# cvg/glue-factory

Measured on AMD Instinct MI355X. Metric: image-pairs/sec (train step) SP+LightGlue N=2048 d=256 L=9, higher is better.
Workload: dtype bf16; 1 GPU; configs[1]: SuperPoint + LightGlue train step -- frozen SuperPoint-open forward on 2x32 synthetic 1024x1024 images resident in HBM (view1 = view0 warped by a sampled homography, SURVEY 8(d)(P); first block and the 64-channel 3x3 blocks as fused HIP kernels, library convolutions + fused HIP tails for the 128/256-channel blocks), homography ground truth (gf_gt_nn), LightGlue fwd + loss + bwd + fused; pairs_per_gpu=32, global_batch=32, keypoints=2048, descriptor_dim=256, layers=9, parallelism=dp1

## Files before the change

### glue-factory_amd/csrc/elementwise.hip

```cpp
#include "gf_common.h"
#include "gf_amd.h"

namespace {

typedef unsigned int u32x4_ __attribute__((ext_vector_type(4)));
__device__ __forceinline__ void load8(float (&x)[8], const bf16_t* p) {
    union { u32x4_ u; bf16_t e[8]; } v;
    v.u = *reinterpret_cast<const u32x4_*>(p);
#pragma unroll
    for (int e = 0; e < 8; ++e) x[e] = (float)v.e[e];
}
__device__ __forceinline__ void load8(float (&x)[8], const float* p) {
    const f32x4 a = *reinterpret_cast<const f32x4*>(p), b = *reinterpret_cast<const f32x4*>(p + 4);
#pragma unroll
    for (int e = 0; e < 4; ++e) { x[e] = a[e]; x[4 + e] = b[e]; }
}
__device__ __forceinline__ void store8(bf16_t* p, const float (&x)[8]) {
    union { u32x4_ u; bf16_t e[8]; } v;
#pragma unroll
    for (int e = 0; e < 8; ++e) v.e[e] = (bf16_t)x[e];
    *reinterpret_cast<u32x4_*>(p) = v.u;
}
__device__ __forceinline__ void store8(float* p, const float (&x)[8]) {
    f32x4 a = {x[0], x[1], x[2], x[3]}, b = {x[4], x[5], x[6], x[7]};
// ... 61 lines not shown
        }
        float acc[4], o[8];
#pragma unroll
        for (int i = 0; i < 4; ++i) {
            const float co = c[2 * i], si = INVERSE ? -c[2 * i + 1] : c[2 * i + 1];
            if (WITH_DTHETA) acc[i] = x[2 * i + 1] * y[2 * i] - x[2 * i] * y[2 * i + 1];
            o[2 * i] = x[2 * i] * co - x[2 * i + 1] * si;
            o[2 * i + 1] = x[2 * i + 1] * co + x[2 * i] * si;
        }
        if (active) store8(base, o);
        if (WITH_DTHETA) {
#pragma unroll
            for (int i = 0; i < 4; ++i)
                for (int off = cpd; off < 64; off <<= 1) acc[i] += __shfl_xor(acc[i], off);
            if (lane < cpd) {
                f32x4 v = {acc[0], acc[1], acc[2], acc[3]};
                if (dtheta_base) v += *reinterpret_cast<const f32x4*>(dtheta_base + tok * (D / 2) + lane * 4);
                *reinterpret_cast<f32x4*>(dtheta + tok * (D / 2) + lane * 4) = v;
            }
        }
    }
}

__device__ __forceinline__ void gelu_parts(float z, float& cdf, float& pdf) {
    const float x = fabsf(z) * 0.70710678118654752f;
    const float t = __builtin_amdgcn_rcpf(1.f + 0.3275911f * x);
    const float e = __expf(-x * x);
    const float poly = t * (0.254829592f + t * (-0.284496736f + t * (1.421413741f + t * (-1.453152027f + t * 1.061405429f))));
    const float erf_abs = 1.f - poly * e;
    cdf = 0.5f * (1.f + copysignf(erf_abs, z));
    pdf = 0.3989422804014327f * e;
}
__device__ __forceinline__ float gelu_f(float z) {
    float cdf, pdf;
    gelu_parts(z, cdf, pdf);
    return z * cdf;
}
__device__ __forceinline__ float gelu_grad(float z) {
    float cdf, pdf;
    gelu_parts(z, cdf, pdf);
    return cdf + z * pdf;
}

template <typename T> struct Chunk { static constexpr int VEC = 16 / sizeof(T); };
typedef unsigned int u32x4 __attribute__((ext_vector_type(4)));

template <typename T, int NCH, bool FULL = false>
__device__ __forceinline__ void load_row(float (&x)[NCH][16 / sizeof(T)], const T* row, int C, int lane) {
    constexpr int VEC = 16 / sizeof(T);
#pragma unroll
    for (int ch = 0; ch < NCH; ++ch) {
        int col = (ch * 64 + lane) * VEC;
        if (FULL || col < C) {
            union { u32x4 u; T e[VEC]; } v;
            v.u = *reinterpret_cast<const u32x4*>(row + col);
#pragma unroll
            for (int e = 0; e < VEC; ++e) x[ch][e] = to_f32(v.e[e]);
        } else {
#pragma unroll
            for (int e = 0; e < VEC; ++e) x[ch][e] = 0.f;
        }
    }
}
template <typename T, int NCH, bool FULL = false>
__device__ __forceinline__ void store_row(T* row, const float (&y)[NCH][16 / sizeof(T)], int C, int lane) {
    constexpr int VEC = 16 / sizeof(T);
// ... 22 lines not shown
            int col = (ch * 64 + lane) * VEC + e;
            g[ch][e] = (FULL || col < C) ? gamma[col] : 0.f;
            bt[ch][e] = (FULL || col < C) ? beta[col] : 0.f;
        }
    constexpr int RPI = 1;
    const int stride = gridDim.x * 4 * RPI;
    const float inv_c = 1.f / C;
    int row = (blockIdx.x * 4 + wave) * RPI;
    float nxt[RPI][NCH][VEC];
#pragma unroll
    for (int r = 0; r < RPI; ++r)
        if (row + r < R) load_row<T, NCH, FULL>(nxt[r], x + (int64_t)(row + r) * C, C, lane);
    for (; row < R; row += stride) {
        float v[RPI][NCH][VEC];
#pragma unroll
        for (int r = 0; r < RPI; ++r)
#pragma unroll
            for (int ch = 0; ch < NCH; ++ch)
#pragma unroll
                for (int e = 0; e < VEC; ++e) v[r][ch][e] = nxt[r][ch][e];
#pragma unroll
        for (int r = 0; r < RPI; ++r)
            if (row + stride + r < R) load_row<T, NCH, FULL>(nxt[r], x + (int64_t)(row + stride + r) * C, C, lane);
        float x0[RPI], s[RPI], q[RPI];
#pragma unroll
        for (int r = 0; r < RPI; ++r) {
            x0[r] = __builtin_bit_cast(float, __builtin_amdgcn_readlane(__builtin_bit_cast(int, v[r][0][0]), 0));
            s[r] = 0.f;
            q[r] = 0.f;
#pragma unroll
            for (int ch = 0; ch < NCH; ++ch)
#pragma unroll
                for (int e = 0; e < VEC; ++e) {
                    int col = (ch * 64 + lane) * VEC + e;
                    float d = (FULL || col < C) ? v[r][ch][e] - x0[r] : 0.f;
                    s[r] += d;
                    q[r] += d * d;
                }
        }
#pragma unroll
        for (int r = 0; r < RPI; ++r) {
            s[r] = wave_allsum(s[r]);
            q[r] = wave_allsum(q[r]);
        }
#pragma unroll
        for (int r = 0; r < RPI; ++r) {
            if (row + r >= R) break;
            const float md = s[r] * inv_c;
            const float mu = x0[r] + md;
            float var = fmaxf(q[r] * inv_c - md * md, 0.f);
            if (md * md > 63.f * var) {
                float q2 = 0.f;
#pragma unroll
                for (int ch = 0; ch < NCH; ++ch)
#pragma unroll
                    for (int e = 0; e < VEC; ++e) {
                        int col = (ch * 64 + lane) * VEC + e;
                        float dc = (FULL || col < C) ? (v[r][ch][e] - x0[r]) - md : 0.f;
                        q2 += dc * dc;
                    }
                var = wave_allsum(q2) * inv_c;
            }
            const float rs = rsqrtf(var + eps);
#pragma unroll
            for (int ch = 0; ch < NCH; ++ch)
#pragma unroll
                for (int e = 0; e < VEC; ++e)
                    v[r][ch][e] = gelu_f((v[r][ch][e] - mu) * rs * g[ch][e] + bt[ch][e]);
            store_row<T, NCH, FULL>(y + (int64_t)(row + r) * C, v[r], C, lane);
            if (lane == 0) { mean[row + r] = mu; rstd[row + r] = rs; }
        }
    }
}

template <typename T, int NCH, bool FULL>
__global__ __launch_bounds__(256) void ln_gelu_bwd_kernel(const T* x, const float* gamma, const float* beta,
                                                          const float* mean, const float* rstd, const T* dy, T* dx,
                                                          float* dgamma_part, float* dbeta_part, int R, int C) {
    constexpr int VEC = 16 / sizeof(T);
    extern __shared__ __attribute__((aligned(16))) char smem[];
    float* red = reinterpret_cast<float*>(smem);
    const int lane = threadIdx.x & 63, wave = threadIdx.x >> 6;
    float g[NCH][VEC], bt[NCH][VEC], dg[NCH][VEC], db[NCH][VEC];
#pragma unroll
    for (int ch = 0; ch < NCH; ++ch)
#pragma unroll
        for (int e = 0; e < VEC; ++e) {
            int col = (ch * 64 + lane) * VEC + e;
            g[ch][e] = (FULL || col < C) ? gamma[col] : 0.f;
            bt[ch][e] = (FULL || col < C) ? beta[col] : 0.f;
            dg[ch][e] = 0.f;
// ... 185 lines not shown
```

### glue-factory_amd/csrc/gemm_st.hip

```cpp
#include <type_traits>
#include "gf_common.h"
#include "gf_amd.h"

namespace {

typedef unsigned int u32x4 __attribute__((ext_vector_type(4)));
typedef unsigned int u32x2 __attribute__((ext_vector_type(2)));
typedef __attribute__((address_space(3))) void gs_lds_void;
typedef const __attribute__((address_space(1))) void gs_glb_void;

constexpr int GS_TILE = 32768;
#ifndef GS_NSTAGE_
#define GS_NSTAGE_ 3
#endif
#ifndef GS_WGS
#define GS_WGS 256
#endif
constexpr int GS_NSTAGE = GS_NSTAGE_, GS_PD = GS_NSTAGE - 1;

struct GsParams {
    const bf16_t* x0; const bf16_t* x1; const bf16_t* w; const float* bias; const bf16_t* res; const bf16_t* res2; bf16_t* y;
    const float* cs;
    int M, N;
    int64_t ld0, ld1, ldw, ldr, ldr2, ldy;
};

template <int OFF> __device__ __forceinline__ u32x4 gs_rd128(unsigned a) {
    u32x4 v;
    asm volatile("ds_read_b128 %0, %1 offset:%2" : "=v"(v) : "v"(a), "n"(OFF) : "memory");
    return v;
}
template <int N> __device__ __forceinline__ void gs_wait_lgkm() { asm volatile("s_waitcnt lgkmcnt(%0)" ::"n"(N) : "memory"); }
template <int N> __device__ __forceinline__ void gs_wait_vm() { asm volatile("s_waitcnt vmcnt(%0)" ::"n"(N) : "memory"); }
template <typename V> __device__ __forceinline__ void gs_tie(V& v) { asm volatile("" : "+v"(v)); }
__device__ __forceinline__ u32x4 gs_ld128(const void* p) {
    u32x4 v;
    asm volatile("global_load_dwordx4 %0, %1, off" : "=v"(v) : "v"(p) : "memory");
    return v;
}
__device__ __forceinline__ void gs_st128(void* p, u32x4 v) {
    asm volatile("global_store_dwordx4 %0, %1, off\n\ts_nop 2" ::"v"(p), "v"(v) : "memory");
}
__device__ __forceinline__ void gs_swap(unsigned& a, unsigned& b) {
    const auto r = __builtin_amdgcn_permlane32_swap(a, b, false, false);
    a = r[0]; b = r[1];
}

template <int KF, bool TWO, int RES, bool ROT>
__global__ __launch_bounds__(512, 2) void gemm_st_kernel(GsParams p) {
    extern __shared__ __attribute__((aligned(1024))) char smem[];
    constexpr int K = 16 * KF, ROWB = 2 * K, CPR = ROWB / 16;
    constexpr int TR = GS_TILE / ROWB, NRB = TR / 32;
    constexpr int NR = RES * 2 * NRB + (ROT ? 4 * NRB : 0), NS = 2 * NRB;
    const unsigned lds0 = (unsigned)(size_t)smem;
    const int lane = threadIdx.x & 63, wave = __builtin_amdgcn_readfirstlane(threadIdx.x >> 6);
    const int l31 = lane & 31, hi = lane >> 5;
    const int ch0 = blockIdx.y * 256 + wave * 32;
    const int ntile = p.M / TR;
    const int T = (ntile - (int)blockIdx.x + (int)gridDim.x - 1) / (int)gridDim.x;
    if (T <= 0) return;

    bf16x8 wf[KF];
#pragma unroll
    for (int s = 0; s < KF; ++s) wf[s] = *reinterpret_cast<const bf16x8*>(p.w + (int64_t)(ch0 + l31) * p.ldw + 16 * s + 8 * hi);
    float bias16[16];
#pragma unroll
    for (int r = 0; r < 16; ++r) bias16[r] = p.bias ? p.bias[ch0 + crow(r, hi)] : 0.f;
    gs_wait_vm<0>();

// ... 180 lines not shown
```

### glue-factory_amd/lib.py

```python
import ctypes
import os
import subprocess

_HERE = os.path.dirname(os.path.abspath(__file__))
LIB_PATH = os.path.join(_HERE, "libgf_amd.so")
CSRC = os.path.join(_HERE, "csrc")
ABI_VERSION = 20

_c = ctypes
_P, _I, _F, _L, _D = _c.c_void_p, _c.c_int, _c.c_float, _c.c_int64, _c.c_double
_S = _c.POINTER(_c.c_int64)

SIGNATURES = {
    "gf_abi_version": [],
    "gf_attn_fwd": [_P, _P, _P, _P, _P, _I, _I, _I, _I, _I, _S, _S, _S, _S, _F, _I, _P],
    "gf_attn_fwd_ex": [_P, _P, _P, _P, _P, _I, _I, _I, _I, _I, _S, _S, _S, _S, _F, _I, _I, _P, _P],
    "gf_attn_cross_bwd": [_P, _P, _P, _P, _P, _P, _P, _P, _I, _I, _I, _I, _I, _S, _S, _S, _S, _S, _S, _F, _I, _P],
    "gf_attn_bwd": [_P, _P, _P, _P, _P, _P, _P, _P, _P, _P, _I, _I, _I, _I, _I,
                    _S, _S, _S, _S, _S, _S, _S, _S, _F, _I, _P],
    "gf_attn_bwd_acc": [_P, _P, _P, _P, _P, _P, _P, _P, _P, _P, _I, _I, _I, _I, _I,
                        _S, _S, _S, _S, _S, _S, _S, _S, _F, _I, _I, _P],
    "gf_rows_lse": [_P, _P, _P, _P, _I, _I, _I, _I, _I, _P],
    "gf_rows_argmax": [_P, _P, _P, _F, _P, _P, _I, _I, _I, _I, _I, _P],
    "gf_assign_write": [_P, _P, _P, _P, _P, _P, _F, _F, _P, _P, _I, _I, _I, _I, _I, _P],
# ... 13 lines not shown
    "gf_line_segsum": [_P, _L, _P, _L, _P, _P, _P, _P, _I, _I, _I, _I, _I, _I, _P],
    "gf_line_expand": [_P, _P, _P, _P, _I, _I, _I, _I, _I, _I, _P],
    "gf_rows_gather": [_P, _P, _P, _I, _I, _I, _I, _I, _P],
    "gf_line_pair_scores": [_P, _P, _P, _I, _I, _I, _I, _P],
    "gf_dense_rowcol": [_P, _L, _L, _P, _P, _I, _I, _I, _I, _P],
    "gf_dense_assign": [_P, _P, _P, _P, _P, _F, _P, _I, _I, _I, _P],
    "gf_dense_assign_bwd": [_P, _P, _P, _P, _P, _P, _P, _I, _I, _I, _P],
    "gf_bgemm": [_P, _P, _P, _I, _I, _I, _I, _S, _S, _S, _F, _I, _P],
    "gf_multi_cast_transpose": [_P, _I, _I, _I, _P],
    "gf_cast_entry_bytes": [],
    "gf_fold_entry_bytes": [],
    "gf_fold_linear_fwd": [_P, _I, _I, _P],
    "gf_fold_linear_bwd": [_P, _P, _P, _P, _P, _P, _P, _P, _P, _I, _I, _I, _I, _I, _P],
    "gf_adam_entry_bytes": [],
    "gf_multi_adam": [_P, _I, _P, _P, _P, _P, _D, _D, _F, _F, _P],
    "gf_weight_grad_map": [_P, _P, _P, _P, _P, _F, _I, _I, _P],
    "gf_colsum_f32": [_P, _P, _P, _I, _I, _I, _P],
    "gf_colsum_ws_floats": [_I, _I],
    "gf_small_dw": [_P, _P, _P, _P, _I, _I, _I, _P],
    "gf_small_dw_ws_floats": [_I, _I],
    "gf_small_fwd": [_P, _P, _P, _I, _I, _I, _P],
    "gf_gemm": [_P, _P, _P, _P, _P, _P, _P, _I, _I, _I, _I, _I, _L, _L, _L, _L, _L, _I, _P],
    "gf_gemm_res2": [_P, _P, _P, _P, _P, _P, _P, _I, _I, _I, _I, _L, _L, _L, _L, _L, _L, _I, _P],
    "gf_linear_dw_ws_bytes": [_I, _I, _I],
    "gf_linear_dw": [_P, _P, _P, _P, _P, _I, _I, _I, _I, _P],
    "gf_linear_dw2": [_P, _P, _P, _I, _P, _P, _P, _I, _I, _I, _I, _P],
    "gf_bn_nblk": [_I],
    "gf_bn_stats": [_P, _P, _I, _I, _I, _P],
    "gf_bn_act_fwd": [_P, _P, _P, _P, _P, _P, _I, _I, _I, _I, _P],
    "gf_bn_bwd_stats": [_P, _P, _P, _P, _P, _P, _P, _I, _I, _I, _I, _P],
    "gf_bn_bwd_dx": [_P, _P, _P, _P, _P, _P, _P, _P, _P, _I, _I, _I, _I, _P],
    "gf_bn_finalize_fwd": [_P, _I, _I, _F, _F, _F, _P, _P, _P, _P, _P, _P],
    "gf_bn_replay_running": [_P, _I, _I, _F, _F, _P, _P, _P, _P],
    "gf_bn_finalize_bwd": [_P, _I, _I, _F, _P, _P, _P, _P, _P],
    "gf_bn_pack_sums": [_P, _I, _I, _I, _F, _P, _P, _P],
    "gf_bn_finalize_sets_fwd": [_P, _I, _I, _F, _F, _P, _P, _P, _P],
    "gf_bn_finalize_sets_bwd": [_P, _P, _I, _I, _P, _P],
    "gf_bn_replay_running_n": [_P, _P, _I, _I, _F, _P, _P, _P, _P],
    "gf_gt_nn": [_P, _P, _P, _P, _P, _P, _P, _I, _I, _I, _P],
    "gf_gt_epi_min": [_P, _P, _P, _P, _P, _P, _I, _I, _I, _P],
    "gf_gt_depth_reward": [_P] * 10 + [_F, _F, _I, _I, _I, _P],
    "gf_line_close_counts": [_P] * 6 + [_I, _I, _I, _I, _F, _I, _P],
    "gf_wf_cluster": [_P] * 8 + [_I, _I, _I, _D, _I, _P],
    "gf_wf_suppress": [_P] * 7 + [_I] * 5 + [_F, _P],
    "gf_wf_descriptors": [_P] * 5 + [_I] * 8 + [_P],
    "gf_wf_associativity": [_P, _P, _I, _I, _I, _P],
# ... 77 lines not shown
```

### glue-factory_amd/matchers/lightglue.py

```python
import math
from pathlib import Path

import torch
import torch.nn.functional as F
from torch import nn

from .. import ops
from ..conf import Conf
from ..metrics import matcher_metrics


def normalize_keypoints(kpts, size=None):
    kpts = kpts.float()
    if size is None:
        size = 1 + kpts.max(-2).values - kpts.min(-2).values
    elif not isinstance(size, torch.Tensor):
        size = torch.tensor(size, device=kpts.device, dtype=kpts.dtype)
    size = size.to(kpts)
    shift = size / 2
    scale = size.max(-1).values / 2
    return (kpts - shift[..., None, :]) / scale[..., None, None]


class _PosEnc(nn.Module):
# ... 7 lines not shown
        w = self.Wr.weight.float()
        theta = ops.small_linear(kpts, w) if kpts.is_cuda else F.linear(kpts, w)
        with torch.no_grad():
            cs = torch.stack((torch.cos(theta), torch.sin(theta)), -1).flatten(-2).contiguous()
        return theta, cs


def _ffn_modules(dim):
    return nn.Sequential(nn.Linear(2 * dim, 2 * dim), nn.LayerNorm(2 * dim, elementwise_affine=True),
                         nn.GELU(), nn.Linear(2 * dim, dim))


def _lin(x, layer):
    if layer.out_features == 1 and layer.in_features % 8 == 0:
        return ops.rowdot(x, layer.weight, layer.bias)[..., None]
    if layer.out_features % 8 or layer.in_features % 8:
        return F.linear(x, layer.weight.to(x.dtype), None if layer.bias is None else layer.bias.to(x.dtype))
    return ops.linear(x, layer.weight, layer.bias)


def _ffn(ffn, x, msg, chain=None, out=None, first=None):
    w0, b0 = (ffn[0].weight, ffn[0].bias) if first is None else first
    h = ops.linear_cat(x, msg, w0, b0, chain1=chain)
    h = ops.ln_gelu(h, ffn[1].weight, ffn[1].bias, ffn[1].eps)
    return ops.linear(h, ffn[3].weight, ffn[3].bias, res=x, res_chain=chain, out=out)


def _fold_spec(name, ffn, proj):
    return (name + ".ffn0", "fold", ffn[0].weight, ffn[0].bias, proj.weight, proj.bias, ffn[0].in_features - proj.out_features, None)


def _folded_ffn0(pc, dtype, ffn, proj):
    if pc is None:
        return None
    return ops.folded_linear(pc[0], dtype, pc[1] + ".ffn0", ffn[0].weight, ffn[0].bias, proj.weight, proj.bias)


class SelfBlock(nn.Module):
    def __init__(self, dim, heads):
        super().__init__()
        self.heads, self.head_dim = heads, dim // heads
        self.Wqkv = nn.Linear(dim, 3 * dim, bias=True)
        self.out_proj = nn.Linear(dim, dim, bias=True)
        self.ffn = _ffn_modules(dim)
        h, c = heads, self.head_dim
        perm = (torch.arange(h)[None, :, None] * (3 * c) + torch.arange(c)[None, None, :] * 3
                + torch.arange(3)[:, None, None]).reshape(-1)
        self.register_buffer("_perm", perm, persistent=False)
# ... 583 lines not shown
```

### glue-factory_amd/ops/__init__.py

```python
from ._base import BF16, F32, _chk, _dt, _p, _s3, _stream
from ._attention import (ATTN_SPLIT, LN2, SharedGradSum, attention, attention_qkv, attn_bwd_raw, attn_fwd_raw, attn_premul,
                         cross_attention, cross_attention_stacked, self_attention_rotary)
from ._params import (_LP_CACHE, _LP_FLAT, _LP_PTR, _LP_T, _DerivedWeight, _lp, _wt_t, derived_weight, folded_linear,
                      invalidate_precast, precast)
from ._linear import (LIBRARY_GEMMS, GradChain, colsum, gemm, gemm_takes, linear, linear_cat, ln_gelu, rowdot, rowdot2,
                      small_linear)
from ._nll import _SPARSE_SUMS, _known_sums, nll_positive_terms, nll_terms
from ._assignment import (_head_bwd, assign_write, bgemm, dual_lse, dual_lse_stacked, filter_matches, lg_layer_loss,
                          n_pair_loss, nn_filter, rows_argmax, rows_lse, rows_top2, similarity)
from ._sinkhorn import sinkhorn, sinkhorn_schedule
from ._batchnorm import (COLLECTIVES, _BatchNormActSetsSync, _ReplayRunningStats, batch_norm_act, batch_norm_act_sets,
                         replay_running_stats)
from ._lines import (_line_graph_sorted, dense_log_double_softmax, line_aggregate, line_gather, line_graph, line_pair_scores,
                     rows_gather)

XBWD_ENABLED = True

FOLD_ENABLED = True

REPLAY_GATE = None

FORCE_SYNC_BN = False
```

### glue-factory_amd/ops/_linear.py

```python
import torch

from .. import lib as _lib
from ._base import _chk, _dt, _p, _stream
from ._params import _lp, _wt_t


_GEMM_KMAX = {torch.bfloat16: 512, torch.float32: 256}


def _k_pieces(k, dtype):
    kmax = _GEMM_KMAX.get(dtype)
    if kmax is None or k < 32:
        return None
    out, rest = [], k
    while rest:
        piece = min(kmax, 1 << (rest.bit_length() - 1))
        if piece < 32:
            return None
        out.append(piece)
        rest -= piece
    return out


def _row_ok(t, dtype):
# ... 452 lines not shown

    @staticmethod
    def backward(ctx, g):
        x, w = ctx.saved_tensors
        O, K = w.shape
        g2, x2 = g.reshape(-1, O).float().contiguous(), x.reshape(-1, K).float().contiguous()
        dx = g @ w if ctx.needs_input_grad[0] else None
        L = _lib.load()
        if not g2.is_cuda or K > 8 or O * K > 256:
            _note_library_gemm(g2.shape[0], O, K, "fp32 (small_linear weight gradient)")
            return dx, (g2.t() @ x2).to(w.dtype)
        ws = torch.empty(L.gf_small_dw_ws_floats(O, K), dtype=torch.float32, device=g2.device)
        dw = torch.empty((O, K), dtype=torch.float32, device=g2.device)
        _lib.check(L.gf_small_dw(_p(g2), _p(x2), _p(ws), _p(dw), g2.shape[0], O, K, _stream()), "gf_small_dw")
        return dx, dw.to(w.dtype)


def small_linear(x, w):
    return _SmallLinear.apply(x, w)


def ln_gelu(x, gamma, beta, eps=1e-5):
    return _LnGelu.apply(x, gamma, beta, eps)
```

### include/gf_amd.h

```cpp
#ifndef GF_AMD_H
#define GF_AMD_H

#include <stdint.h>

#ifdef __cplusplus
extern "C" {
#endif

#define GF_DTYPE_F32 0
#define GF_DTYPE_BF16 1

#define GF_ERR_UNSUPPORTED (-1)
#define GF_ERR_SHAPE (-2)
#define GF_ERR_ALIGN (-3)
#define GF_ERR_DTYPE (-4)

#define GF_AMD_ABI_VERSION 20
int gf_abi_version(void);

int gf_attn_fwd(const void* q, const void* k, const void* v, void* o, float* lse,
                int B, int H, int Nq, int Nk, int D,
                const int64_t* q_strides, const int64_t* k_strides,
                const int64_t* v_strides, const int64_t* o_strides,
                float scale, int dtype, void* stream);
// ... 104 lines not shown
                       float* dW0, float* dWo, float* dbo, int R, int K, int N, int ldw0, int c0, void* stream);
int gf_cast_entry_bytes(void);
int gf_weight_grad_map(const float* g, float* out, const int* perm, const int* cperm, const float* rscale, float scale,
                       int rows, int cols, void* stream);
int gf_colsum_f32(const float* x, float* ws, float* out, int G, int R, int C, void* stream);
int gf_colsum_ws_floats(int G, int C);
int gf_small_dw(const float* dy, const float* x, float* ws, float* dw, int M, int O, int K, void* stream);
int gf_small_dw_ws_floats(int O, int K);
int gf_small_fwd(const float* x, const float* w, float* y, int M, int O, int K, void* stream);
int gf_adam_entry_bytes(void);
int gf_multi_adam(const void* table, int n_entries, const float* lr, float* step, const float* found_inf,
                  const float* grad_scale, double beta1, double beta2, float eps, float weight_decay, void* stream);

int gf_bgemm(const void* a, const void* b, void* c, int batch, int M, int N, int K,
             const int64_t* a_strides, const int64_t* b_strides, const int64_t* c_strides,
             float alpha, int dtype, void* stream);

int gf_gemm(const void* x0, const void* x1, const void* w, const float* bias, const void* res, void* y,
            const float* cs, int rot_n, int M, int N, int K0, int K1,
            int64_t ld0, int64_t ld1, int64_t ldw, int64_t ldr, int64_t ldy, int dtype, void* stream);
int gf_gemm_res2(const void* x0, const void* x1, const void* w, const float* bias, const void* res, const void* res_b,
                 void* y, int M, int N, int K0, int K1, int64_t ld0, int64_t ld1, int64_t ldw, int64_t ldr,
                 int64_t ldr_b, int64_t ldy, int dtype, void* stream);

int64_t gf_linear_dw_ws_bytes(int M, int Nout, int K);
int gf_linear_dw(const void* dy, const void* x, float* dw, float* db, void* ws,
                 int M, int Nout, int K, int dtype, void* stream);
int gf_linear_dw2(const void* dy, const void* x1, const void* x2, int K1, float* dw, float* db, void* ws,
                  int M, int Nout, int K, int dtype, void* stream);

int gf_bn_nblk(int M);
int gf_bn_stats(const void* x, float* part, int M, int C, int dtype, void* stream);
int gf_bn_act_fwd(const void* x, const float* mean, const float* rstd, const float* gamma,
                  const float* beta, void* y, int M, int C, int relu, int dtype, void* stream);
int gf_bn_bwd_stats(const void* x, const void* dy, const float* mean, const float* rstd,
                    const float* gamma, const float* beta, float* part, int M, int C, int relu,
                    int dtype, void* stream);
int gf_bn_bwd_dx(const void* x, const void* dy, const float* mean, const float* rstd,
                 const float* gamma, const float* beta, const float* m1, const float* m2,
                 void* dx, int M, int C, int relu, int dtype, void* stream);
int gf_bn_finalize_fwd(const float* part, int nblk, int C, float n, float eps, float momentum,
                       float* mean, float* var, float* rstd, float* run_mean, float* run_var, void* stream);
int gf_bn_finalize_bwd(const float* part, int nblk, int C, float n, float* dbeta, float* dgamma,
                       float* m1, float* m2, void* stream);
int gf_bn_pack_sums(const float* part, int sets, int nblk, int C, float n_local, float* packed, float* local_copy,
                    void* stream);
// ... 105 lines not shown
```

Measured before the change: 530.5 image-pairs/s.

## Fuse FFN LayerNorm+GELU into the second FFN linear GEMM kernel

Adds a new persistent GEMM kernel that loads the FFN hidden tile into LDS, applies LayerNorm+GELU in place (also writing the activated tensor, mean and rstd for backward), then runs the MFMA GEMM with bias and residual on it. The goal is to avoid a separate ln_gelu launch and the extra HBM round trip of reading the activation back for the GEMM. Waves are split so that half do the LN of the next tile before their MMA and half after, overlapping LN with matrix work. A shared header is factored out, and the path is gated to bf16 K=512, N=256, with fallback to the old two-kernel path.

```diff
diff --git a/glue-factory_amd/csrc/elementwise.hip b/glue-factory_amd/csrc/elementwise.hip
--- a/glue-factory_amd/csrc/elementwise.hip
+++ b/glue-factory_amd/csrc/elementwise.hip
@@ -1,5 +1,6 @@
 #include "gf_common.h"
 #include "gf_amd.h"
+#include "ln_gelu_math.h"
 
 namespace {
 
@@ -107,26 +108,6 @@
     }
 }
 
-__device__ __forceinline__ void gelu_parts(float z, float& cdf, float& pdf) {
-    const float x = fabsf(z) * 0.70710678118654752f;
-    const float t = __builtin_amdgcn_rcpf(1.f + 0.3275911f * x);
-    const float e = __expf(-x * x);
-    const float poly = t * (0.254829592f + t * (-0.284496736f + t * (1.421413741f + t * (-1.453152027f + t * 1.061405429f))));
-    const float erf_abs = 1.f - poly * e;
-    cdf = 0.5f * (1.f + copysignf(erf_abs, z));
-    pdf = 0.3989422804014327f * e;
-}
-__device__ __forceinline__ float gelu_f(float z) {
-    float cdf, pdf;
-    gelu_parts(z, cdf, pdf);
-    return z * cdf;
-}
-__device__ __forceinline__ float gelu_grad(float z) {
-    float cdf, pdf;
-    gelu_parts(z, cdf, pdf);
-    return cdf + z * pdf;
-}
-
 template <typename T> struct Chunk { static constexpr int VEC = 16 / sizeof(T); };
 typedef unsigned int u32x4 __attribute__((ext_vector_type(4)));
 
@@ -195,51 +176,11 @@
 #pragma unroll
         for (int r = 0; r < RPI; ++r)
             if (row + stride + r < R) load_row<T, NCH, FULL>(nxt[r], x + (int64_t)(row + stride + r) * C, C, lane);
-        float x0[RPI], s[RPI], q[RPI];
-#pragma unroll
-        for (int r = 0; r < RPI; ++r) {
-            x0[r] = __builtin_bit_cast(float, __builtin_amdgcn_readlane(__builtin_bit_cast(int, v[r][0][0]), 0));
-            s[r] = 0.f;
-            q[r] = 0.f;
-#pragma unroll
-            for (int ch = 0; ch < NCH; ++ch)
-#pragma unroll
-                for (int e = 0; e < VEC; ++e) {
-                    int col = (ch * 64 + lane) * VEC + e;
-                    float d = (FULL || col < C) ? v[r][ch][e] - x0[r] : 0.f;
-                    s[r] += d;
-                    q[r] += d * d;
-                }
-        }
-#pragma unroll
-        for (int r = 0; r < RPI; ++r) {
-            s[r] = wave_allsum(s[r]);
-            q[r] = wave_allsum(q[r]);
-        }
 #pragma unroll
         for (int r = 0; r < RPI; ++r) {
             if (row + r >= R) break;
-            const float md = s[r] * inv_c;
-            const float mu = x0[r] + md;
-            float var = fmaxf(q[r] * inv_c - md * md, 0.f);
-            if (md * md > 63.f * var) {
-                float q2 = 0.f;
-#pragma unroll
-                for (int ch = 0; ch < NCH; ++ch)
-#pragma unroll
-                    for (int e = 0; e < VEC; ++e) {
-                        int col = (ch * 64 + lane) * VEC + e;
-                        float dc = (FULL || col < C) ? (v[r][ch][e] - x0[r]) - md : 0.f;
-                        q2 += dc * dc;
-                    }
-                var = wave_allsum(q2) * inv_c;
-            }
-            const float rs = rsqrtf(var + eps);
-#pragma unroll
-            for (int ch = 0; ch < NCH; ++ch)
-#pragma unroll
-                for (int e = 0; e < VEC; ++e)
-                    v[r][ch][e] = gelu_f((v[r][ch][e] - mu) * rs * g[ch][e] + bt[ch][e]);
+            float mu, rs;
+            ln_gelu_row<NCH, VEC, FULL>(v[r], g, bt, C, lane, inv_c, eps, mu, rs);
             store_row<T, NCH, FULL>(y + (int64_t)(row + r) * C, v[r], C, lane);
             if (lane == 0) { mean[row + r] = mu; rstd[row + r] = rs; }
         }
diff --git a/glue-factory_amd/csrc/gemm_st.hip b/glue-factory_amd/csrc/gemm_st.hip
--- a/glue-factory_amd/csrc/gemm_st.hip
+++ b/glue-factory_amd/csrc/gemm_st.hip
@@ -1,22 +1,9 @@
 #include <type_traits>
 #include "gf_common.h"
 #include "gf_amd.h"
+#include "gemm_st_common.h"
 
 namespace {
-
-typedef unsigned int u32x4 __attribute__((ext_vector_type(4)));
-typedef unsigned int u32x2 __attribute__((ext_vector_type(2)));
-typedef __attribute__((address_space(3))) void gs_lds_void;
-typedef const __attribute__((address_space(1))) void gs_glb_void;
-
-constexpr int GS_TILE = 32768;
-#ifndef GS_NSTAGE_
-#define GS_NSTAGE_ 3
-#endif
-#ifndef GS_WGS
-#define GS_WGS 256
-#endif
-constexpr int GS_NSTAGE = GS_NSTAGE_, GS_PD = GS_NSTAGE - 1;
 
 struct GsParams {
     const bf16_t* x0; const bf16_t* x1; const bf16_t* w; const float* bias; const bf16_t* res; const bf16_t* res2; bf16_t* y;
@@ -24,27 +11,6 @@
     int M, N;
     int64_t ld0, ld1, ldw, ldr, ldr2, ldy;
 };
-
-template <int OFF> __device__ __forceinline__ u32x4 gs_rd128(unsigned a) {
-    u32x4 v;
-    asm volatile("ds_read_b128 %0, %1 offset:%2" : "=v"(v) : "v"(a), "n"(OFF) : "memory");
-    return v;
-}
-template <int N> __device__ __forceinline__ void gs_wait_lgkm() { asm volatile("s_waitcnt lgkmcnt(%0)" ::"n"(N) : "memory"); }
-template <int N> __device__ __forceinline__ void gs_wait_vm() { asm volatile("s_waitcnt vmcnt(%0)" ::"n"(N) : "memory"); }
-template <typename V> __device__ __forceinline__ void gs_tie(V& v) { asm volatile("" : "+v"(v)); }
-__device__ __forceinline__ u32x4 gs_ld128(const void* p) {
-    u32x4 v;
-    asm volatile("global_load_dwordx4 %0, %1, off" : "=v"(v) : "v"(p) : "memory");
-    return v;
-}
-__device__ __forceinline__ void gs_st128(void* p, u32x4 v) {
-    asm volatile("global_store_dwordx4 %0, %1, off\n\ts_nop 2" ::"v"(p), "v"(v) : "memory");
-}
-__device__ __forceinline__ void gs_swap(unsigned& a, unsigned& b) {
-    const auto r = __builtin_amdgcn_permlane32_swap(a, b, false, false);
-    a = r[0]; b = r[1];
-}
 
 template <int KF, bool TWO, int RES, bool ROT>
 __global__ __launch_bounds__(512, 2) void gemm_st_kernel(GsParams p) {
diff --git a/glue-factory_amd/csrc/gemm_st_common.h b/glue-factory_amd/csrc/gemm_st_common.h
--- /dev/null
+++ b/glue-factory_amd/csrc/gemm_st_common.h
@@ -0,0 +1,41 @@
+#pragma once
+#include "gf_common.h"
+
+namespace {
+
+typedef unsigned int u32x4 __attribute__((ext_vector_type(4)));
+typedef unsigned int u32x2 __attribute__((ext_vector_type(2)));
+typedef __attribute__((address_space(3))) void gs_lds_void;
+typedef const __attribute__((address_space(1))) void gs_glb_void;
+
+constexpr int GS_TILE = 32768;
+#ifndef GS_NSTAGE_
+#define GS_NSTAGE_ 3
+#endif
+#ifndef GS_WGS
+#define GS_WGS 256
+#endif
+constexpr int GS_NSTAGE = GS_NSTAGE_, GS_PD = GS_NSTAGE - 1;
+
+template <int OFF> __device__ __forceinline__ u32x4 gs_rd128(unsigned a) {
+    u32x4 v;
+    asm volatile("ds_read_b128 %0, %1 offset:%2" : "=v"(v) : "v"(a), "n"(OFF) : "memory");
+    return v;
+}
+template <int N> __device__ __forceinline__ void gs_wait_lgkm() { asm volatile("s_waitcnt lgkmcnt(%0)" ::"n"(N) : "memory"); }
+template <int N> __device__ __forceinline__ void gs_wait_vm() { asm volatile("s_waitcnt vmcnt(%0)" ::"n"(N) : "memory"); }
+template <typename V> __device__ __forceinline__ void gs_tie(V& v) { asm volatile("" : "+v"(v)); }
+__device__ __forceinline__ u32x4 gs_ld128(const void* p) {
+    u32x4 v;
+    asm volatile("global_load_dwordx4 %0, %1, off" : "=v"(v) : "v"(p) : "memory");
+    return v;
+}
+__device__ __forceinline__ void gs_st128(void* p, u32x4 v) {
+    asm volatile("global_store_dwordx4 %0, %1, off\n\ts_nop 2" ::"v"(p), "v"(v) : "memory");
+}
+__device__ __forceinline__ void gs_swap(unsigned& a, unsigned& b) {
+    const auto r = __builtin_amdgcn_permlane32_swap(a, b, false, false);
+    a = r[0]; b = r[1];
+}
+
+}
diff --git a/glue-factory_amd/csrc/gemm_st_ln.hip b/glue-factory_amd/csrc/gemm_st_ln.hip
--- /dev/null
+++ b/glue-factory_amd/csrc/gemm_st_ln.hip
@@ -0,0 +1,247 @@
+#include <type_traits>
+#include "gf_common.h"
+#include "gf_amd.h"
+#include "gemm_st_common.h"
+#include "ln_gelu_math.h"
+
+namespace {
+
+struct GlParams {
+    const bf16_t* x; const bf16_t* w; const float* bias; const bf16_t* res; bf16_t* y;
+    const float* gamma; const float* beta; bf16_t* hact; float* mean; float* rstd;
+    float eps;
+    int M;
+    int64_t ldx, ldw, ldr, ldy;
+};
+
+__device__ __forceinline__ void gl_lds_st128(unsigned a, u32x4 v) {
+    asm volatile("ds_write_b128 %0, %1" ::"v"(a), "v"(v) : "memory");
+}
+__device__ __forceinline__ void gl_st32(void* p, float v) {
+    asm volatile("global_store_dword %0, %1, off" ::"v"(p), "v"(v) : "memory");
+}
+
+__global__ __launch_bounds__(512, 2) void gemm_ln_gelu_kernel(GlParams p) {
+    extern __shared__ __attribute__((aligned(1024))) char smem[];
+    constexpr int KF = 32, K = 16 * KF, ROWB = 2 * K, CPR = ROWB / 16;
+    constexpr int TR = GS_TILE / ROWB;
+    constexpr int NR = 2, ND = 4, NL = 4 + 2, NS = 2;
+    constexpr int PER = NR + ND + NL + NS;
+    constexpr int GL_NSTAGE = 4, GL_PD = GL_NSTAGE - 1;
+    static_assert(TR == 32 && CPR == 64, "a wave owns 4 whole rows of a tile, a lane one chunk of a row");
+    const unsigned lds0 = (unsigned)(size_t)smem;
+    const int lane = threadIdx.x & 63, wave = __builtin_amdgcn_readfirstlane(threadIdx.x >> 6);
+    const int l31 = lane & 31, hi = lane >> 5;
+    const int ch0 = wave * 32;
+    const int ntile = p.M / TR;
+    const int T = (ntile - (int)blockIdx.x + (int)gridDim.x - 1) / (int)gridDim.x;
+    if (T <= 0) return;
+
+    bf16x8 wf[KF];
+#pragma unroll
+    for (int s = 0; s < KF; ++s) wf[s] = *reinterpret_cast<const bf16x8*>(p.w + (int64_t)(ch0 + l31) * p.ldw + 16 * s + 8 * hi);
+    float bias16[16];
+#pragma unroll
+    for (int r = 0; r < 16; ++r) bias16[r] = p.bias ? p.bias[ch0 + crow(r, hi)] : 0.f;
+    {
+        float* gb = reinterpret_cast<float*>(smem + GL_NSTAGE * GS_TILE);
+        const int t = threadIdx.x;
+        if (t < 256) *reinterpret_cast<f32x4*>(gb + 4 * t) = *reinterpret_cast<const f32x4*>(t < 128 ? p.gamma + 4 * t : p.beta + 4 * (t - 128));
+    }
+    __syncthreads();
+    const unsigned gba = lds0 + (unsigned)(GL_NSTAGE * GS_TILE + 32 * lane);
+    gs_wait_vm<0>();
+
+    auto issue = [&](int i, int stage) {
+        const int ti = (int)blockIdx.x + min(i, T - 1) * (int)gridDim.x;
+#pragma unroll
+        for (int j = 0; j < 4; ++j) {
+            const int piece = 4 * wave + j;
+            const int lin = 64 * piece + lane;
+            const int row = lin / CPR, c = (lin % CPR) ^ (row & 15);
+            const int64_t grow = (int64_t)ti * TR + row;
+            const bf16_t* src = p.x + grow * p.ldx + c * 8;
+            __builtin_amdgcn_global_load_lds((gs_glb_void*)src, (gs_lds_void*)(smem + stage * GS_TILE + piece * 1024), 16, 0, 0);
+        }
+    };
+#pragma unroll
+    for (int t = 0; t < GL_PD; ++t) issue(t, t);
+
+    unsigned a0[8];
+#pragma unroll
+    for (int sl = 0; sl < 8; ++sl) a0[sl] = lds0 + (unsigned)(l31 * ROWB + (((2 * sl + hi) ^ (l31 & 15)) << 4));
+    const int64_t ycol = ch0 + 8 * hi;
+    const float inv_c = 1.f / K;
+
+    auto ln_tile = [&](int stage, int64_t r0) {
+        unsigned la[4];
+        u32x4 raw[4];
+#pragma unroll
+        for (int j = 0; j < 4; ++j) {
+            const int row = 4 * wave + j;
+            la[j] = lds0 + (unsigned)(stage * GS_TILE + row * ROWB + ((lane ^ (row & 15)) << 4));
+            raw[j] = gs_rd128<0>(la[j]);
+        }
+        u32x4 gq[4] = {gs_rd128<0>(gba), gs_rd128<16>(gba), gs_rd128<4 * K>(gba), gs_rd128<4 * K + 16>(gba)};
+        gs_wait_lgkm<0>();
+        __builtin_amdgcn_sched_barrier(0);
+        float g[1][8], bt[1][8];
+#pragma unroll
+        for (int q = 0; q < 4; ++q) gs_tie(gq[q]);
+#pragma unroll
+        for (int e = 0; e < 4; ++e) {
+            g[0][e] = __builtin_bit_cast(f32x4, gq[0])[e]; g[0][4 + e] = __builtin_bit_cast(f32x4, gq[1])[e];
+            bt[0][e] = __builtin_bit_cast(f32x4, gq[2])[e]; bt[0][4 + e] = __builtin_bit_cast(f32x4, gq[3])[e];
+        }
+        float mu[4], rs[4];
+#pragma unroll
+        for (int j = 0; j < 4; ++j) {
+            gs_tie(raw[j]);
+            const bf16x8 hb = __builtin_bit_cast(bf16x8, raw[j]);
+            float v[1][8];
+#pragma unroll
+            for (int e = 0; e < 8; ++e) v[0][e] = (float)hb[e];
+            ln_gelu_row<1, 8, true>(v, g, bt, K, lane, inv_c, p.eps, mu[j], rs[j]);
+            const bf16x8 ob = {(bf16_t)v[0][0], (bf16_t)v[0][1], (bf16_t)v[0][2], (bf16_t)v[0][3],
+                               (bf16_t)v[0][4], (bf16_t)v[0][5], (bf16_t)v[0][6], (bf16_t)v[0][7]};
+            const u32x4 o = __builtin_bit_cast(u32x4, ob);
+            gl_lds_st128(la[j], o);
+            gs_st128(p.hact + (r0 + 4 * wave + j) * K + 8 * lane, o);
+        }
+        float mv = mu[0], rv = rs[0];
+#pragma unroll
+        for (int j = 1; j < 4; ++j) { mv = lane == j ? mu[j] : mv; rv = lane == j ? rs[j] : rv; }
+        if (lane < 4) {
+            gl_st32(p.mean + r0 + 4 * wave + lane, mv);
+            gl_st32(p.rstd + r0 + 4 * wave + lane, rv);
+        }
+    };
+    f32x16 acc;
+    auto mma_tile = [&](int stage) {
+        unsigned a[8];
+#pragma unroll
+        for (int sl = 0; sl < 8; ++sl) a[sl] = a0[sl] + stage * GS_TILE;
+        u32x4 xa[4], xb[4];
+        auto rd = [&](u32x4 (&dst)[4], auto G) {
+            constexpr int gq = decltype(G)::value;
+#pragma unroll
+            for (int q = 0; q < 4; ++q) dst[q] = gs_rd128<((4 * gq) / 8) * 256>(a[(4 * gq + q) & 7]);
+        };
+        auto mma = [&](u32x4 (&src)[4], auto G) {
+            constexpr int gq = decltype(G)::value;
+#pragma unroll
+            for (int q = 0; q < 4; ++q) {
+                gs_tie(src[q]);
+                acc = __builtin_amdgcn_mfma_f32_32x32x16_bf16(wf[4 * gq + q], __builtin_bit_cast(bf16x8, src[q]), acc, 0, 0, 0);
+            }
+        };
+        constexpr int NG = KF / 4;
+#pragma unroll
+        for (int r = 0; r < 16; ++r) acc[r] = bias16[r];
+        rd(xa, std::integral_constant<int, 0>{});
+        rd(xb, std::integral_constant<int, 1>{});
+        auto step = [&](u32x4 (&buf)[4], auto G) {
+            constexpr int gq = decltype(G)::value;
+            if constexpr (gq == NG - 1) gs_wait_lgkm<0>(); else gs_wait_lgkm<4>();
+            mma(buf, G);
+            if constexpr (gq + 2 < NG) rd(buf, std::integral_constant<int, gq + 2>{});
+        };
+        step(xa, std::integral_constant<int, 0>{}); step(xb, std::integral_constant<int, 1>{});
+        step(xa, std::integral_constant<int, 2>{}); step(xb, std::integral_constant<int, 3>{});
+        step(xa, std::integral_constant<int, 4>{}); step(xb, std::integral_constant<int, 5>{});
+        step(xa, std::integral_constant<int, 6>{}); step(xb, std::integral_constant<int, 7>{});
+    };
+    auto store_tile = [&](int64_t r0, u32x4 (&rr)[2]) {
+        bf16_t* yp = p.y + (r0 + l31) * p.ldy + ycol;
+#pragma unroll
+        for (int j = 0; j < 2; ++j) {
+            float v[2][4];
+#pragma unroll
+            for (int e = 0; e < 4; ++e) { v[0][e] = acc[8 * j + e]; v[1][e] = acc[8 * j + 4 + e]; }
+            gs_tie(rr[j]);
+            unsigned a0_ = rr[j][0], a1_ = rr[j][1], b0_ = rr[j][2], b1_ = rr[j][3];
+            gs_swap(a0_, b0_);
+            gs_swap(a1_, b1_);
+            const bf16x4 r0_ = __builtin_bit_cast(bf16x4, u32x2{a0_, a1_}), r1_ = __builtin_bit_cast(bf16x4, u32x2{b0_, b1_});
+#pragma unroll
+            for (int e = 0; e < 4; ++e) { v[0][e] += (float)r0_[e]; v[1][e] += (float)r1_[e]; }
+            const bf16x4 o0 = {(bf16_t)v[0][0], (bf16_t)v[0][1], (bf16_t)v[0][2], (bf16_t)v[0][3]};
+            const bf16x4 o1 = {(bf16_t)v[1][0], (bf16_t)v[1][1], (bf16_t)v[1][2], (bf16_t)v[1][3]};
+            const u32x2 p0 = __builtin_bit_cast(u32x2, o0), p1 = __builtin_bit_cast(u32x2, o1);
+            unsigned q0 = p0[0], q1 = p0[1], q2 = p1[0], q3 = p1[1];
+            gs_swap(q0, q2);
+            gs_swap(q1, q3);
+            gs_st128(yp + 16 * j, u32x4{q0, q1, q2, q3});
+        }
+    };
+    auto tile_row0 = [&](int i) { return ((int64_t)blockIdx.x + (int64_t)i * gridDim.x) * TR; };
+
+    gs_wait_vm<(GL_PD - 1) * ND>();
+    ln_tile(0, tile_row0(0));
+    gs_wait_lgkm<0>();
+    const bool ln_first = wave < 4;
+
+    for (int i = 0; i < T; ++i) {
+        const int64_t row0 = tile_row0(i);
+        const bool more = i + 1 < T;
+        __builtin_amdgcn_s_barrier();
+        __builtin_amdgcn_sched_barrier(0);
+        u32x4 rr[2];
+#pragma unroll
+        for (int j = 0; j < 2; ++j) rr[j] = gs_ld128(p.res + (row0 + l31) * p.ldr + ycol + 16 * j);
+        issue(i + GL_PD, (i + GL_PD) % GL_NSTAGE);
+        if (ln_first) {
+            if (more) {
+                if (i >= 2) gs_wait_vm<NL + NS + PER + NR + ND>();
+                else if (i == 1) gs_wait_vm<NL + PER + NR + ND>();
+                else gs_wait_vm<ND + NL + NR + ND>();
+                ln_tile((i + 1) % GL_NSTAGE, tile_row0(i + 1));
+            }
+            __builtin_amdgcn_sched_barrier(0);
+            mma_tile(i % GL_NSTAGE);
+            if (more) gs_wait_vm<ND + NL>(); else gs_wait_vm<ND>();
+            __builtin_amdgcn_sched_barrier(0);
+            store_tile(row0, rr);
+        } else {
+            mma_tile(i % GL_NSTAGE);
+            gs_wait_vm<ND>();
+            __builtin_amdgcn_sched_barrier(0);
+            store_tile(row0, rr);
+            __builtin_amdgcn_sched_barrier(0);
+            if (more) {
+                if (i >= 2) gs_wait_vm<NS + NL + PER + NR + ND + NS>();
+                else if (i == 1) gs_wait_vm<NL + PER + NR + ND + NS>();
+                else gs_wait_vm<ND + NL + NR + ND + NS>();
+                ln_tile((i + 1) % GL_NSTAGE, tile_row0(i + 1));
+                gs_wait_lgkm<0>();
+            }
+        }
+    }
+    gs_wait_vm<0>();
+}
+
+}
+
+extern "C" int gf_gemm_ln_gelu(const void* h, const float* gamma, const float* beta, float eps, const void* w,
+                               const float* bias, const void* res, void* y, void* h_act, float* mean, float* rstd,
+                               int M, int N, int K, int64_t ldh, int64_t ldw, int64_t ldr, int64_t ldy, int dtype,
+                               void* stream) {
+    if (dtype != GF_BF16 || K != 512 || N != 256 || M <= 0 || M % 64) return GF_ERR_UNSUPPORTED;
+    if (!h || !gamma || !beta || !w || !res || !y || !h_act || !mean || !rstd) return GF_ERR_UNSUPPORTED;
+    if (ldh < K || ldw < K || ldr < N || ldy < N || ldh % 8 || ldw % 8 || ldr % 8 || ldy % 8) return GF_ERR_UNSUPPORTED;
+    if (((uintptr_t)h | (uintptr_t)w | (uintptr_t)res | (uintptr_t)y | (uintptr_t)h_act) % 16) return GF_ERR_UNSUPPORTED;
+    GlParams p;
+    p.x = static_cast<const bf16_t*>(h); p.w = static_cast<const bf16_t*>(w); p.bias = bias;
+    p.res = static_cast<const bf16_t*>(res); p.y = static_cast<bf16_t*>(y);
+    p.gamma = gamma; p.beta = beta; p.hact = static_cast<bf16_t*>(h_act); p.mean = mean; p.rstd = rstd;
+    p.eps = eps; p.M = M; p.ldx = ldh; p.ldw = ldw; p.ldr = ldr; p.ldy = ldy;
+    hipStream_t st = reinterpret_cast<hipStream_t>(stream);
+    const size_t lds = (size_t)4 * GS_TILE + 2 * 512 * sizeof(float);
+    hipError_t e = hipFuncSetAttribute(reinterpret_cast<const void*>(gemm_ln_gelu_kernel),
+                                       hipFuncAttributeMaxDynamicSharedMemorySize, (int)lds);
+    if (e != hipSuccess) return (int)e;
+    const int ntile = M / 32;
+    const int gx = GS_WGS < ntile ? GS_WGS : ntile;
+    gemm_ln_gelu_kernel<<<dim3(gx), dim3(512), lds, st>>>(p);
+    return (int)hipGetLastError();
+}
diff --git a/glue-factory_amd/csrc/ln_gelu_math.h b/glue-factory_amd/csrc/ln_gelu_math.h
--- /dev/null
+++ b/glue-factory_amd/csrc/ln_gelu_math.h
@@ -0,0 +1,61 @@
+#pragma once
+#include "gf_common.h"
+
+__device__ __forceinline__ void gelu_parts(float z, float& cdf, float& pdf) {
+    const float x = fabsf(z) * 0.70710678118654752f;
+    const float t = __builtin_amdgcn_rcpf(1.f + 0.3275911f * x);
+    const float e = __expf(-x * x);
+    const float poly = t * (0.254829592f + t * (-0.284496736f + t * (1.421413741f + t * (-1.453152027f + t * 1.061405429f))));
+    const float erf_abs = 1.f - poly * e;
+    cdf = 0.5f * (1.f + copysignf(erf_abs, z));
+    pdf = 0.3989422804014327f * e;
+}
+__device__ __forceinline__ float gelu_f(float z) {
+    float cdf, pdf;
+    gelu_parts(z, cdf, pdf);
+    return z * cdf;
+}
+__device__ __forceinline__ float gelu_grad(float z) {
+    float cdf, pdf;
+    gelu_parts(z, cdf, pdf);
+    return cdf + z * pdf;
+}
+
+template <int NCH, int VEC, bool FULL>
+__device__ __forceinline__ void ln_gelu_row(float (&v)[NCH][VEC], const float (&g)[NCH][VEC], const float (&bt)[NCH][VEC],
+                                            int C, int lane, float inv_c, float eps, float& mu, float& rs) {
+    const float x0 = __builtin_bit_cast(float, __builtin_amdgcn_readlane(__builtin_bit_cast(int, v[0][0]), 0));
+    float s = 0.f, q = 0.f;
+#pragma unroll
+    for (int ch = 0; ch < NCH; ++ch)
+#pragma unroll
+        for (int e = 0; e < VEC; ++e) {
+            int col = (ch * 64 + lane) * VEC + e;
+            float d = (FULL || col < C) ? v[ch][e] - x0 : 0.f;
+            s += d;
+            q += d * d;
+        }
+    s = wave_allsum(s);
+    q = wave_allsum(q);
+    const float md = s * inv_c;
+    mu = x0 + md;
+    float var = fmaxf(q * inv_c - md * md, 0.f);
+    if (md * md > 63.f * var) {
+        float q2 = 0.f;
+#pragma unroll
+        for (int ch = 0; ch < NCH; ++ch)
+#pragma unroll
+            for (int e = 0; e < VEC; ++e) {
+                int col = (ch * 64 + lane) * VEC + e;
+                float dc = (FULL || col < C) ? (v[ch][e] - x0) - md : 0.f;
+                q2 += dc * dc;
+            }
+        var = wave_allsum(q2) * inv_c;
+    }
+    rs = rsqrtf(var + eps);
+#pragma unroll
+    for (int ch = 0; ch < NCH; ++ch)
+#pragma unroll
+        for (int e = 0; e < VEC; ++e)
+            v[ch][e] = gelu_f((v[ch][e] - mu) * rs * g[ch][e] + bt[ch][e]);
+}
diff --git a/glue-factory_amd/lib.py b/glue-factory_amd/lib.py
--- a/glue-factory_amd/lib.py
+++ b/glue-factory_amd/lib.py
@@ -59,6 +59,7 @@
     "gf_small_fwd": [_P, _P, _P, _I, _I, _I, _P],
     "gf_gemm": [_P, _P, _P, _P, _P, _P, _P, _I, _I, _I, _I, _I, _L, _L, _L, _L, _L, _I, _P],
     "gf_gemm_res2": [_P, _P, _P, _P, _P, _P, _P, _I, _I, _I, _I, _L, _L, _L, _L, _L, _L, _I, _P],
+    "gf_gemm_ln_gelu": [_P, _P, _P, _F, _P, _P, _P, _P, _P, _P, _P, _I, _I, _I, _L, _L, _L, _L, _I, _P],
     "gf_linear_dw_ws_bytes": [_I, _I, _I],
     "gf_linear_dw": [_P, _P, _P, _P, _P, _I, _I, _I, _I, _P],
     "gf_linear_dw2": [_P, _P, _P, _I, _P, _P, _P, _I, _I, _I, _I, _P],
diff --git a/glue-factory_amd/matchers/lightglue.py b/glue-factory_amd/matchers/lightglue.py
--- a/glue-factory_amd/matchers/lightglue.py
+++ b/glue-factory_amd/matchers/lightglue.py
@@ -53,8 +53,7 @@
 def _ffn(ffn, x, msg, chain=None, out=None, first=None):
     w0, b0 = (ffn[0].weight, ffn[0].bias) if first is None else first
     h = ops.linear_cat(x, msg, w0, b0, chain1=chain)
-    h = ops.ln_gelu(h, ffn[1].weight, ffn[1].bias, ffn[1].eps)
-    return ops.linear(h, ffn[3].weight, ffn[3].bias, res=x, res_chain=chain, out=out)
+    return ops.linear_ln_gelu(h, ffn[1].weight, ffn[1].bias, ffn[1].eps, ffn[3].weight, ffn[3].bias, x, res_chain=chain, out=out)
 
 
 def _fold_spec(name, ffn, proj):
diff --git a/glue-factory_amd/ops/__init__.py b/glue-factory_amd/ops/__init__.py
--- a/glue-factory_amd/ops/__init__.py
+++ b/glue-factory_amd/ops/__init__.py
@@ -3,8 +3,8 @@
                          cross_attention, cross_attention_stacked, self_attention_rotary)
 from ._params import (_LP_CACHE, _LP_FLAT, _LP_PTR, _LP_T, _DerivedWeight, _lp, _wt_t, derived_weight, folded_linear,
                       invalidate_precast, precast)
-from ._linear import (LIBRARY_GEMMS, GradChain, colsum, gemm, gemm_takes, linear, linear_cat, ln_gelu, rowdot, rowdot2,
-                      small_linear)
+from ._linear import (LIBRARY_GEMMS, GradChain, colsum, ffn_fused_takes, gemm, gemm_takes, linear, linear_cat, linear_ln_gelu,
+                      ln_gelu, rowdot, rowdot2, small_linear)
 from ._nll import _SPARSE_SUMS, _known_sums, nll_positive_terms, nll_terms
 from ._assignment import (_head_bwd, assign_write, bgemm, dual_lse, dual_lse_stacked, filter_matches, lg_layer_loss,
                           n_pair_loss, nn_filter, rows_argmax, rows_lse, rows_top2, similarity)
@@ -18,6 +18,8 @@
 
 FOLD_ENABLED = True
 
+FFN_FUSED = True
+
 REPLAY_GATE = None
 
 FORCE_SYNC_BN = False
diff --git a/glue-factory_amd/ops/_linear.py b/glue-factory_amd/ops/_linear.py
--- a/glue-factory_amd/ops/_linear.py
+++ b/glue-factory_amd/ops/_linear.py
@@ -498,3 +498,98 @@
 
 def ln_gelu(x, gamma, beta, eps=1e-5):
     return _LnGelu.apply(x, gamma, beta, eps)
+
+
+def _ln_gelu_gemm(h2, g32, b32, eps, wt, bias, res2, out2):
+    M, K = h2.shape
+    N = wt.shape[0]
+    L = _lib.load()
+    y = torch.empty((M, N), dtype=h2.dtype, device=h2.device) if out2 is None else out2
+    h_act = torch.empty((M, K), dtype=h2.dtype, device=h2.device)
+    mean = torch.empty(M, dtype=torch.float32, device=h2.device)
+    rstd = torch.empty(M, dtype=torch.float32, device=h2.device)
+    rc = -1
+    if res2 is not None and wt.dtype == h2.dtype and res2.dtype == h2.dtype and h2.dtype in (torch.bfloat16, torch.float32):
+        bias32 = None if bias is None else bias.detach().float().contiguous()
+        rc = L.gf_gemm_ln_gelu(_p(h2), _p(g32), _p(b32), float(eps), _p(wt), _p(bias32), _p(res2), _p(y), _p(h_act), _p(mean),
+                               _p(rstd), M, N, K, h2.stride(0), wt.stride(0), res2.stride(0), y.stride(0), _dt(h2), _stream())
+    if rc == -1:
+        _lib.check(L.gf_ln_gelu_fwd(_p(h2), _p(g32), _p(b32), _p(h_act), _p(mean), _p(rstd), M, K, float(eps), _dt(h2),
+                                    _stream()), "gf_ln_gelu_fwd")
+        y = _linear_fwd(h_act, wt, bias, res2, out=out2)
+    else:
+        _lib.check(rc, "gf_gemm_ln_gelu")
+    return y, h_act, mean, rstd
+
+
+class _LnGeluLinear(torch.autograd.Function):
+
+    @staticmethod
+    def forward(ctx, h, gamma, beta, eps, w, b, res, res_chain, out):
+        _chk(h, gamma, beta)
+        ctx.res_chain = res_chain
+        wt = _lp(w, h.dtype)
+        K = h.shape[-1]
+        h2 = h.reshape(-1, K)
+        if not h2.is_contiguous():
+            h2 = h2.contiguous()
+        res2 = res.reshape(-1, wt.shape[0])
+        if not res2.is_contiguous():
+            res2 = res2.contiguous()
+        out2 = None if out is None else out.view(-1, wt.shape[0])
+        g32, b32 = gamma.float().contiguous(), beta.float().contiguous()
+        y, h_act, mean, rstd = _ln_gelu_gemm(h2, g32, b32, eps, wt, b, res2, out2)
+        ctx.save_for_backward(h2, h_act, mean, rstd, g32, b32, wt)
+        ctx.shape = h.shape
+        ctx.dtypes = (gamma.dtype, beta.dtype, w.dtype, None if b is None else b.dtype)
+        return y.view(*h.shape[:-1], wt.shape[0])
+
+    @staticmethod
+    def backward(ctx, dy):
+        h2, h_act, mean, rstd, g32, b32, wt = ctx.saved_tensors
+        nout, k = wt.shape
+        M = h2.shape[0]
+        dy2 = dy.reshape(-1, nout)
+        if not dy2.is_contiguous():
+            dy2 = dy2.contiguous()
+        dres = dy if ctx.needs_input_grad[6] else None
+        if dres is not None and ctx.res_chain is not None:
+            d2 = _flat2(dres, nout)
+            rc = ctx.res_chain
+            if rc.acc is not None:
+                if rc.extra is not None:
+                    d2 = d2 + rc.pop_extra()
+                rc.extra = rc.acc
+            rc.park(d2)
+            dres = None
+        dh = dg = dbt = dw = db = None
+        need_ln = any(ctx.needs_input_grad[:3])
+        d_act = gemm(dy2, _wt_t(wt)) if need_ln else None
+        if ctx.needs_input_grad[4] or (ctx.dtypes[3] is not None and ctx.needs_input_grad[5]):
+            dw32, db32 = _dw(dy2, h_act, nout, k, ctx.dtypes[3] is not None)
+            dw = dw32.to(ctx.dtypes[2])
+            db = None if db32 is None else db32.to(ctx.dtypes[3])
+        if need_ln:
+            L = _lib.load()
+            nblk = L.gf_ln_gelu_nblk(M)
+            dh = torch.empty_like(h2)
+            part = torch.empty((2, nblk, k), dtype=torch.float32, device=h2.device)
+            _lib.check(L.gf_ln_gelu_bwd(_p(h2), _p(g32), _p(b32), _p(mean), _p(rstd), _p(d_act), _p(dh),
+                                        _p(part[0]), _p(part[1]), M, k, _dt(h2), _stream()), "gf_ln_gelu_bwd")
+            sums = colsum(part)
+            dh, dg, dbt = dh.view(ctx.shape), sums[0].to(ctx.dtypes[0]), sums[1].to(ctx.dtypes[1])
+        return dh, dg, dbt, None, dw, db, dres, None, None
+
+
+def ffn_fused_takes(h, w):
+    from . import FFN_FUSED
+    return bool(FFN_FUSED) and h.is_cuda and h.dtype == torch.bfloat16 and h.shape[-1] == 512 and tuple(w.shape) == (256, 512)
+
+
+def linear_ln_gelu(h, gamma, beta, eps, w, b, res, res_chain=None, out=None):
+    if not ffn_fused_takes(h, w):
+        return linear(ln_gelu(h, gamma, beta, eps), w, b, res=res, res_chain=res_chain, out=out)
+    _chk(h, res)
+    if not res.requires_grad:
+        res_chain = None
+    return _LnGeluLinear.apply(h, gamma, beta, eps, w, b, res, res_chain, out)
diff --git a/include/gf_amd.h b/include/gf_amd.h
--- a/include/gf_amd.h
+++ b/include/gf_amd.h
@@ -150,6 +150,9 @@
 int gf_gemm_res2(const void* x0, const void* x1, const void* w, const float* bias, const void* res, const void* res_b,
                  void* y, int M, int N, int K0, int K1, int64_t ld0, int64_t ld1, int64_t ldw, int64_t ldr,
                  int64_t ldr_b, int64_t ldy, int dtype, void* stream);
+int gf_gemm_ln_gelu(const void* h, const float* gamma, const float* beta, float eps, const void* w, const float* bias,
+                    const void* res, void* y, void* h_act, float* mean, float* rstd, int M, int N, int K,
+                    int64_t ldh, int64_t ldw, int64_t ldr, int64_t ldy, int dtype, void* stream);
 
 int64_t gf_linear_dw_ws_bytes(int M, int Nout, int K);
 int gf_linear_dw(const void* dy, const void* x, float* dw, float* db, void* ws,
```

Result: no change. 531.5 image-pairs/s, median of 6 (+0.2%).
